# pema99/rust-path-tracer

Hardware: AMD Instinct MI355X
Metric: Mrays/s (higher is better)
Workload: dtype f32

## Files before the change

### rust-path-tracer_amd/csrc/k_traverse_nearest.h

```cpp
#ifndef RPT_K_TRAVERSE_NEAREST_H
#define RPT_K_TRAVERSE_NEAREST_H

#include "k_path.h"
#include "k_walk_stream.h"

template <int STACK, int THREADS>
__global__ __launch_bounds__(THREADS) void k_traverse_nearest(DevScene sc, DevState st, DevQueues q, uint32_t iteration) {
    __shared__ uint32_t lds_stack[THREADS / RPT_WAVE][STACK][RPT_WAVE];
    if (q.count[Q_DRAINED] != 0u) return;
    const uint32_t slot = blockIdx.x * THREADS + threadIdx.x;
    if (slot == 0u) {
        iteration_bookkeeping(q, iteration);
    }
    bool pending = false;
    if (slot < st.n_slots) pending = __float_as_uint(st.hit[slot].y) == HIT_PENDING;
    const SceneViewGlobal view{{sc.tri_isect}, sc.nodes};
    unsigned long long active = rpt_ballot(pending);
    if (active == 0ull) return;
    if (__lane_id() == (uint32_t)__ffsll((long long)active) - 1u) {
        raise_flag(&q.count[Q_ALIVE0 + (iteration & 1u) * Q_LINE]);
        atomicAdd(&q.ray_shards[(blockIdx.x % RPT_STAT_SHARDS) * RPT_STAT_STRIDE], (unsigned long long)__popcll(active));
    }
    if (!pending) return;
    float4 ra = st.ray_a[slot];
    float2 rb = st.ray_b[slot];
    F3 ro = f3(ra.x, ra.y, ra.z), rd = f3(ra.w, rb.x, rb.y);
    uint32_t *stack = &lds_stack[threadIdx.x / RPT_WAVE][0][threadIdx.x % RPT_WAVE];
    HitRecord h = traverse_one<STACK, false>(view, sc.fastdiv_ok, ro, rd, 0.0f, stack);
    store_hit(st, slot, h);
}

#define RPT_NEAREST_PLAIN 0
#define RPT_NEAREST_LAST 1
#define RPT_NEAREST_FIRST 2
template <int STACK, int THREADS, int MODE = RPT_NEAREST_PLAIN>
__attribute__((amdgpu_num_sgpr(RPT_LDS_WALK_SGPRS)))
__global__ __launch_bounds__(THREADS) void k_traverse_nearest_stream(DevScene sc, DevState st, DevQueues q, uint32_t iteration,
                                                                       uint32_t SPAN ,
                                                                       float cam_x, float cam_y, float cam_z ,
                                                                       DevConfig cfg, uint32_t gen_samples ,
                                                                       DevStats *stats) {
    constexpr bool LAST = MODE == RPT_NEAREST_LAST, FIRST = MODE == RPT_NEAREST_FIRST;
    constexpr uint32_t NW = THREADS / RPT_WAVE;
    __shared__ uint16_t lds_stack[NW][STACK][RPT_WAVE];
    __shared__ WgPool pool;
    float4 *lds_scene = rpt_lds_dyn;
    if (q.count[Q_DRAINED] != 0u) return;
    uint32_t *global_next = &q.count[Q_POOL0 + (iteration & 1u) * Q_LINE];
    if (blockIdx.x == 0u && threadIdx.x == 0u) {
        iteration_bookkeeping(q, iteration);
        q.count[Q_POOL0 + ((iteration + 1u) & 1u) * Q_LINE] = 0u;
    }
    const uint32_t lane = __lane_id(), wave = threadIdx.x / RPT_WAVE;
    if (threadIdx.x == 0u) {
        const uint32_t g = atomicAdd(global_next, SPAN);
        pool.word = wg_pool_span(g, SPAN, st.n_slots);
        pool.lock = 0u;
    }
    __syncthreads();
    if ((uint32_t)(pool.word >> 32) == 0u) return;
    if (LAST)
        for (uint32_t k = threadIdx.x; k < sc.last_flip_vecs; k += THREADS) lds_scene[sc.lds_vecs + k] = sc.lds_image_last[k];
    if (FIRST) {
        const uint32_t P2 = 2u * sc.lds_pairs;
        for (uint32_t k = threadIdx.x; k < 3u * P2; k += THREADS) {
            const float4 v = sc.lds_image[k];
            const float o = k < P2 ? cam_x : (k < 2u * P2 ? cam_y : cam_z);
            lds_scene[k] = make_float4(v.x - o, v.y - o, v.z - o, v.w - o);
        }
        for (uint32_t k = 3u * P2 + threadIdx.x; k < sc.lds_vecs; k += THREADS) lds_scene[k] = sc.lds_image[k];
        __syncthreads();
    }
    const SceneViewLds view = FIRST ? SceneViewLds{lds_scene, sc.lds_pairs, sc.n_triangles, sc.lds_root} : stage_scene_lds<THREADS>(sc, lds_scene);
    const float4 *img_lane = view.img;
    uint32_t stop_first = 0u;
    float order_bias = 0.0f;
    uint16_t *stack = &lds_stack[wave][0][lane];
    F3 ro = f3(0, 0, 0), rd = f3(1, 1, 1), ird = f3(1, 1, 1);
    LdsWalk w;
    walk_begin(view, w);
    w.cur = SceneViewLds::dead();
    uint32_t slot = 0u;
    bool have = false;
    bool pool_open = true;
    uint32_t traced = 0u;
    const bool done_here = LAST && q.implicit_zero != 0u;
    auto last_finish = [&](uint32_t s, const HitRecord &r, uint32_t stopped) -> bool {
        if (!done_here) {
            store_hit(st, s, r);
            return false;
        }
        if (r.tri == HIT_MISS) return true;
        if (stopped == 0u) {
            const uint32_t m = __float_as_uint(sc.tri_shade[4u * (r.tri & 0x7fffffffu) + 2u].w);
            const float4 e4 = sc.textured != 0u ? sc.materials[6u * m] : sc.mat_lite[2u * m];
            if ((e4.x != 0.0f || e4.y != 0.0f || e4.z != 0.0f) && (r.tri >> 31) == 0u) {
                const float4 tf = st.thr[s];
                finish_from_zero(st, s, mask_nan3(f3(tf.x, tf.y, tf.z) * f3(e4.x, e4.y, e4.z)));
                return false;
            }
        }
        set_hit_word(st, s, HIT_DONE_ZERO);
        return false;
    };
    auto last_park = [&](bool park, uint32_t s) {
        const uint32_t shard = (s >> q.sky_shard_shift) % RPT_Q_SHARDS;
        unsigned long long todo_m = rpt_ballot(park);
        while (todo_m != 0ull) {
            const uint32_t leader = (uint32_t)__ffsll((long long)todo_m) - 1u;
            const uint32_t sh = (uint32_t)__builtin_amdgcn_readlane((int)shard, (int)leader);
            const bool mine = park && shard == sh;
            const unsigned long long same = rpt_ballot(mine);
            uint32_t e = 0u;
            if (lane == leader) e = atomicAdd(&q.sky_cnt[sh * RPT_Q_SHARD_STRIDE], (uint32_t)__popcll(same));
            e = (uint32_t)__builtin_amdgcn_readlane((int)e, (int)leader);
            if (mine) {
                e += rpt_lane_rank(same);
                q.sky[q_position(sh, e)] = s;
                set_hit_word(st, s, HIT_PARKED);
            }
            todo_m &= ~same;
        }
    };
    for (;;) {
        const unsigned long long idle_m = rpt_ballot(walk_dead(w));
        const uint32_t n_idle = (uint32_t)__popcll(idle_m);
        if (pool_open && n_idle >= (uint32_t)RPT_STREAM_REFILL) {
            uint32_t base = 0u, got = 0u;
            bool finished = false;
            if (lane == 0u) base = wg_pool_take(&pool, global_next, st.n_slots, SPAN, n_idle, got, finished);
            base = (uint32_t)__builtin_amdgcn_readfirstlane((int)base);
            got = (uint32_t)__builtin_amdgcn_readfirstlane((int)got);
            pool_open = __builtin_amdgcn_readfirstlane((int)finished) == 0;
            bool took = false;
            if (LAST) {
                const bool writes = walk_dead(w) && have;
                bool park = false;
                if (writes) {
                    park = last_finish(slot, w.res, stop_first);
                    have = false;
                }
                if (done_here) last_park(park, slot);
            }
            if (walk_dead(w)) {
                if (!LAST && have) {
                    store_hit(st, slot, w.res);
                    have = false;
                }
                const uint32_t rank = rpt_lane_rank(idle_m);
                if (rank < got) {
                    const uint32_t cand = base + rank;
                    const uint32_t word = __float_as_uint(st.hit[cand].y);
                    bool pending;
                    if (FIRST && gen_samples != 0u) {
                        pending = begin_first_path(st, cfg, stats, cand, word, gen_samples, ro, rd);
                    } else {
                        pending = word == HIT_PENDING;
                        if (pending) {
                            const float4 ra = st.ray_a[cand];
                            const float2 rb = st.ray_b[cand];
                            ro = f3(ra.x, ra.y, ra.z); rd = f3(ra.w, rb.x, rb.y);
                        }
                    }
                    if (pending) {
                        slot = cand;
                        took = true;
                        if (fastdiv_ray_ok(sc.fastdiv_ok, ro, rd)) {
                            ird = f3(rptm::rcp_rn_window(rd.x), rptm::rcp_rn_window(rd.y), rptm::rcp_rn_window(rd.z));
                            walk_begin(view, w);
                            have = true;
                            if (LAST) {
                                bool may_emit = false;
                                for (uint32_t e = 0; e < sc.last_emit_n; ++e) {
                                    float t_e;
                                    bool bf_e;
                                    may_emit = moller_trumbore_view(view, sc.last_emit_tri[e], ro, rd, t_e, bf_e) || may_emit;
                                }
                                stop_first = may_emit ? 0u : 1u;
                                const bool flipped = !may_emit && sc.last_flip_vecs != 0u;
                                img_lane = flipped ? view.img + sc.lds_vecs : view.img;
                                order_bias = flipped ? __builtin_inff() : 0.0f;
                            }
                        } else {
                            LdsWalk alone;
                            walk_begin(view, alone);
                            lds_walk_run<STACK, false, false, false, false, FIRST>(view, alone, ro, rd, rd, 0.0f, stack, 0x7fffffff);
                            if (LAST) {
                                w.res = alone.res;
                                stop_first = 0u;
                                have = true;
                            } else {
                                store_hit(st, cand, alone.res);
                            }
                        }
                    }
                }
            }
            traced += (uint32_t)__popcll(rpt_ballot(took));
            if (got != 0u || !pool_open) continue;
            if (idle_m == ~0ull) { __builtin_amdgcn_s_sleep(8); continue; }
        }
        if (idle_m == ~0ull) {
            if (!pool_open) break;
            continue;
        }
        if (LAST) lds_walk_run<STACK, false, true, false, true>(view, w, ro, rd, ird, 0.0f, stack, pool_open ? RPT_STREAM_TRIPS : 0x7fffffff, img_lane, stop_first, order_bias);
        else lds_walk_run<STACK, false, true, false, false, FIRST>(view, w, ro, rd, ird, 0.0f, stack, pool_open ? RPT_STREAM_TRIPS : 0x7fffffff);
    }
    if (LAST) {
        bool park = false;
        if (have) park = last_finish(slot, w.res, stop_first);
        if (done_here) last_park(park, slot);
    } else if (have) {
        store_hit(st, slot, w.res);
    }
    if (lane == 0u && traced != 0u) {
        raise_flag(&q.count[Q_ALIVE0 + (iteration & 1u) * Q_LINE]);
        atomicAdd(&q.ray_shards[(blockIdx.x % RPT_STAT_SHARDS) * RPT_STAT_STRIDE], (unsigned long long)traced);
    }
}

template <int STACK, int WIDTH , bool COOP >
__attribute__((amdgpu_waves_per_eu(gstream_waves(STACK, WIDTH, COOP), 8)))
 __global__ __launch_bounds__(RPT_WAVE) void k_traverse_nearest_gstream(DevScene sc, DevState st, DevQueues q, uint32_t iteration,
                                                                       uint32_t SPAN ) {
    __shared__ WaveStack<STACK, WIDTH> lds_stack;
    __shared__ uint16_t pend[RPT_WAVE * gstream_rays_nearest(STACK, WIDTH)];
    if (q.count[Q_DRAINED] != 0u) return;
    const uint32_t lane = threadIdx.x;
    if (blockIdx.x == 0u && lane == 0u) {
        iteration_bookkeeping(q, iteration);
    }
    const uint32_t span_begin = blockIdx.x * SPAN;
    if (span_begin >= st.n_slots) return;
    const uint32_t span_end = span_begin + SPAN < st.n_slots ? span_begin + SPAN : st.n_slots;
    uint32_t count = 0u;
    for (uint32_t base = span_begin; base < span_end; base += RPT_WAVE) {
        const uint32_t s = base + lane;
        const bool p = s < span_end && __float_as_uint(st.hit[s].y) == HIT_PENDING;
        const unsigned long long m = rpt_ballot(p);
        if (p) pend[count + rpt_lane_rank(m)] = (uint16_t)(s - span_begin);
        count += (uint32_t)__popcll(m);
    }
    if (count == 0u) return;
    __builtin_amdgcn_fence(__ATOMIC_RELEASE, "wavefront");
    __builtin_amdgcn_wave_barrier();
    if (lane == 0u) {
        raise_flag(&q.count[Q_ALIVE0 + (iteration & 1u) * Q_LINE]);
        atomicAdd(&q.ray_shards[(blockIdx.x % RPT_STAT_SHARDS) * RPT_STAT_STRIDE], (unsigned long long)count);
    }
    typedef SceneViewPairsT<COOP> View;
    const View view{{sc.tri_isect}, sc.gpairs, sc.glinks};
    auto stack = lds_stack.column(lane);
    F3 ro = f3(0, 0, 0), rd = f3(1, 1, 1), ird = f3(1, 1, 1);
    Walk<View> w;
    walk_begin(view, w);
    w.cur = View::dead();
    uint32_t slot = 0u, next = 0u;
    bool have = false;
    const uint32_t refill_at = iteration == 0u ? (uint32_t)RPT_GSTREAM_REFILL_FIRST : (uint32_t)RPT_GSTREAM_REFILL;
    for (;;) {
        const unsigned long long idle_m = rpt_ballot(walk_dead(w));
        const uint32_t n_idle = (uint32_t)__popcll(idle_m);
        const bool more = next < count;
        if ((more && n_idle >= refill_at) || idle_m == ~0ull) {
            if (walk_dead(w)) {
                if (have) {
                    store_hit(st, slot, w.res);
                    have = false;
                }
                const uint32_t at = next + rpt_lane_rank(idle_m);
                if (at < count) {
                    slot = span_begin + pend[at];
                    const float4 ra = st.ray_a[slot];
                    const float2 rb = st.ray_b[slot];
                    ro = f3(ra.x, ra.y, ra.z); rd = f3(ra.w, rb.x, rb.y);
                    have = true;
                    if (fastdiv_ray_ok(sc.fastdiv_ok, ro, rd)) {
                        ird = f3(rptm::rcp_rn_window(rd.x), rptm::rcp_rn_window(rd.y), rptm::rcp_rn_window(rd.z));
                        walk_begin(view, w);
                    } else {
                        w.res = traverse_loop<STACK, false, false>(view, ro, rd, rd, 0.0f, stack);
                    }
                }
            }
            if (!more) break;
            next += n_idle;
            continue;
        }
        walk_run<STACK, false, true>(view, w, ro, rd, ird, 0.0f, stack, more ? RPT_GSTREAM_TRIPS : 0x7fffffff);
    }
}

#endif
```

### rust-path-tracer_amd/csrc/k_traverse_shadow_kernels.h

```cpp
template <int STACK, int THREADS>
__global__ __launch_bounds__(THREADS) void RPT_SHADOW_KERNEL(k_traverse_shadow)(DevScene sc, DevState st, DevQueues q, DevConfig cfg, DevStats *stats) {
    constexpr bool SEGMENT = RPT_SHADOW_KERNEL_SEGMENT;
    __shared__ uint32_t lds_stack[THREADS / RPT_WAVE][STACK][RPT_WAVE];
    if (q.count[Q_DRAINED] != 0u) return;
    uint32_t i = blockIdx.x * THREADS + threadIdx.x;
    uint32_t positions, n;
    q_extent(q.shadow_cnt, positions, n);
    if (i == 0u && n) atomicAdd(&stats->shadow_rays, (unsigned long long)n);
    if (blockIdx.x * THREADS >= positions) return;
    const SceneViewGlobal view{{sc.tri_isect}, sc.nodes};
    if (i >= positions || !q_filled(q.shadow_cnt, i)) return;
    float4 o = q.sh_o[i], d = q.sh_d[i];
    uint32_t tag = __float_as_uint(d.w);
    uint32_t *stack = &lds_stack[threadIdx.x / RPT_WAVE][0][threadIdx.x % RPT_WAVE];
    HitRecord h = traverse_one<STACK, true, SEGMENT>(view, sc.fastdiv_ok, f3(o.x, o.y, o.z), f3(d.x, d.y, d.z), SEGMENT ? shadow_segment_bound(o.w) : o.w, stack);
    shadow_resolve(st, q, cfg, i, tag, h.tri == HIT_MISS);
}

template <int STACK, int THREADS, bool FIXED >
__attribute__((amdgpu_num_sgpr(RPT_LDS_WALK_SGPRS)))
__global__ __launch_bounds__(THREADS) void RPT_SHADOW_KERNEL(k_traverse_shadow_stream)(DevScene sc, DevState st, DevQueues q, DevStats *stats, uint32_t SPAN) {
    constexpr bool SEGMENT = RPT_SHADOW_KERNEL_SEGMENT;
    constexpr uint32_t NW = THREADS / RPT_WAVE;
    __shared__ uint16_t lds_stack[NW][STACK][RPT_WAVE];
    __shared__ WgPool pool;
    float4 *lds_scene = rpt_lds_dyn;
    if (q.count[Q_DRAINED] != 0u) return;
    uint32_t n, n_entries;
    q_extent(q.shadow_cnt, n, n_entries);
    uint32_t *global_next = &q.count[Q_SPOOL];
    if (blockIdx.x == 0u && threadIdx.x == 0u && n_entries) atomicAdd(&stats->shadow_rays, (unsigned long long)n_entries);
    const uint32_t lane = __lane_id(), wave = threadIdx.x / RPT_WAVE;
    if (threadIdx.x == 0u) {
        const uint32_t g = n ? atomicAdd(global_next, SPAN) : 0u;
        pool.word = wg_pool_span(g, SPAN, n);
        pool.lock = 0u;
    }
    __syncthreads();
    if ((uint32_t)(pool.word >> 32) == 0u) return;
    const SceneViewLds view = stage_scene_lds<THREADS>(sc, lds_scene, FIXED);
    uint16_t *stack = &lds_stack[wave][0][lane];
    F3 ro = f3(0, 0, 0), rd = f3(1, 1, 1), ird = f3(1, 1, 1);
    float max_t = 0.0f;
    LdsWalk w;
    walk_begin(view, w);
    w.cur = SceneViewLds::dead();
    uint32_t entry = 0u;
    bool have = false;
    bool pool_open = true;
    for (;;) {
        const unsigned long long idle_m = rpt_ballot(walk_dead(w));
        const uint32_t n_idle = (uint32_t)__popcll(idle_m);
        if (pool_open && n_idle >= (uint32_t)RPT_STREAM_REFILL) {
            uint32_t base = 0u, got = 0u;
            bool finished = false;
            if (lane == 0u) base = wg_pool_take(&pool, global_next, n, SPAN, n_idle, got, finished);
            base = (uint32_t)__builtin_amdgcn_readfirstlane((int)base);
            got = (uint32_t)__builtin_amdgcn_readfirstlane((int)got);
            pool_open = __builtin_amdgcn_readfirstlane((int)finished) == 0;
            if (walk_dead(w)) {
                if (have) {
                    q.sh_c[entry].w = w.res.tri == HIT_MISS ? 0.0f : 1.0f;
                    have = false;
                }
                const uint32_t rank = rpt_lane_rank(idle_m);
                if (rank < got && q_filled(q.shadow_cnt, base + rank)) {
                    entry = base + rank;
                    const float4 o = q.sh_o[entry], d = q.sh_d[entry];
                    ro = f3(o.x, o.y, o.z); rd = f3(d.x, d.y, d.z);
                    max_t = SEGMENT ? shadow_segment_bound(o.w) : o.w;
                    have = true;
                    if (fastdiv_ray_ok(sc.fastdiv_ok, ro, rd)) {
                        ird = f3(rptm::rcp_rn_window(rd.x), rptm::rcp_rn_window(rd.y), rptm::rcp_rn_window(rd.z));
                        walk_begin(view, w);
                    } else {
                        w.res = traverse_loop<STACK, true, false, FIXED, SEGMENT>(view, ro, rd, rd, max_t, stack);
                    }
                }
            }
            if (got != 0u || !pool_open) continue;
            if (idle_m == ~0ull) { __builtin_amdgcn_s_sleep(8); continue; }
        }
        if (idle_m == ~0ull) {
            if (!pool_open) break;
            continue;
        }
        lds_walk_run<STACK, true, true, FIXED, false, false, SEGMENT>(view, w, ro, rd, ird, max_t, stack, pool_open ? RPT_STREAM_TRIPS : 0x7fffffff);
    }
    if (have) q.sh_c[entry].w = w.res.tri == HIT_MISS ? 0.0f : 1.0f;
}

template <int STACK, int WIDTH, bool COOP, bool FIXED >
__attribute__((amdgpu_waves_per_eu(gstream_waves(STACK, WIDTH, COOP), 8)))
 __global__ __launch_bounds__(RPT_WAVE) void RPT_SHADOW_KERNEL(k_traverse_shadow_gstream)(DevScene sc, DevState st, DevQueues q, DevConfig cfg, DevStats *stats,
                                                                      uint32_t SPAN) {
    constexpr bool SEGMENT = RPT_SHADOW_KERNEL_SEGMENT;
    __shared__ WaveStack<STACK, WIDTH> lds_stack;
    __shared__ uint8_t occluded[RPT_WAVE * RPT_GSTREAM_RAYS];
    if (q.count[Q_DRAINED] != 0u) return;
    const uint32_t lane = threadIdx.x;
    uint32_t n, n_entries;
    q_extent(q.shadow_cnt, n, n_entries);
    if (blockIdx.x == 0u && lane == 0u && n_entries) atomicAdd(&stats->shadow_rays, (unsigned long long)n_entries);
    const uint32_t begin = blockIdx.x * SPAN;
    if (begin >= n) return;
    const uint32_t end = begin + SPAN < n ? begin + SPAN : n;
    {
        typedef SceneViewPairsT<COOP> View;
        const View view = FIXED ? View{{sc.tri_isect}, sc.gpairs_shadow, sc.glinks_shadow} : View{{sc.tri_isect}, sc.gpairs, sc.glinks};
        auto stack = lds_stack.column(lane);
        F3 ro = f3(0, 0, 0), rd = f3(1, 1, 1), ird = f3(1, 1, 1);
        float max_t = 0.0f;
        Walk<View> w;
        walk_begin(view, w);
        w.cur = View::dead();
        uint32_t entry = 0u, next = begin;
        bool have = false;
        for (;;) {
            const unsigned long long idle_m = rpt_ballot(walk_dead(w));
            const uint32_t n_idle = (uint32_t)__popcll(idle_m);
            const bool more = next < end;
            if ((more && n_idle >= (uint32_t)RPT_GSTREAM_REFILL) || idle_m == ~0ull) {
                if (walk_dead(w)) {
                    if (have) {
                        occluded[entry - begin] = w.res.tri == HIT_MISS ? (uint8_t)0 : (uint8_t)1;
                        have = false;
                    }
                    const uint32_t at = next + rpt_lane_rank(idle_m);
                    if (at < end && q_filled(q.shadow_cnt, at)) {
                        const float4 o = q.sh_o[at], d = q.sh_d[at];
                        ro = f3(o.x, o.y, o.z); rd = f3(d.x, d.y, d.z);
                        max_t = SEGMENT ? shadow_segment_bound(o.w) : o.w;
                        entry = at;
                        have = true;
                        if (fastdiv_ray_ok(sc.fastdiv_ok, ro, rd)) {
                            ird = f3(rptm::rcp_rn_window(rd.x), rptm::rcp_rn_window(rd.y), rptm::rcp_rn_window(rd.z));
                            walk_begin(view, w);
                        } else {
                            w.res = traverse_loop<STACK, true, false, FIXED, SEGMENT>(view, ro, rd, rd, max_t, stack);
                        }
                    }
                }
                if (!more) break;
                next += n_idle;
                continue;
            }
            walk_run<STACK, true, true, FIXED, SEGMENT>(view, w, ro, rd, ird, max_t, stack, more ? RPT_GSTREAM_TRIPS : 0x7fffffff);
        }
    }
    __builtin_amdgcn_fence(__ATOMIC_RELEASE, "wavefront");
    __builtin_amdgcn_wave_barrier();
    for (uint32_t base = begin; base < end; base += RPT_WAVE) {
        const uint32_t e = base + lane;
        if (e < end && q_filled(q.shadow_cnt, e)) shadow_resolve(st, q, cfg, e, __float_as_uint(q.sh_d[e].w), occluded[e - begin] == 0u);
    }
}

template <int STACK, bool ANY_HIT, bool LDS_SCENE, int THREADS>
__global__ __launch_bounds__(THREADS) void RPT_SHADOW_KERNEL(k_trace_debug)(DevScene sc, uint32_t n, const float *origins, const float *dirs,
                                                         const float *max_t, float *out_t, uint32_t *out_tri, uint32_t *out_flags) {
    constexpr bool SEGMENT = RPT_SHADOW_KERNEL_SEGMENT && ANY_HIT;
    typedef typename StackElem<LDS_SCENE>::type StackT;
    __shared__ StackT lds_stack[THREADS / RPT_WAVE][STACK][RPT_WAVE];
    float4 *lds_scene = rpt_lds_dyn;
    uint32_t i = blockIdx.x * THREADS + threadIdx.x;
    const auto view = stage_scene<LDS_SCENE, THREADS>(sc, lds_scene);
    if (i >= n) return;
    F3 ro = f3(origins[3 * i], origins[3 * i + 1], origins[3 * i + 2]);
    F3 rd = f3(dirs[3 * i], dirs[3 * i + 1], dirs[3 * i + 2]);
    StackT *stack = &lds_stack[threadIdx.x / RPT_WAVE][0][threadIdx.x % RPT_WAVE];
    HitRecord h = traverse_one<STACK, ANY_HIT, SEGMENT>(view, sc.fastdiv_ok, ro, rd, ANY_HIT ? (SEGMENT ? shadow_segment_bound(max_t[i]) : max_t[i]) : 0.0f, stack);
    out_t[i] = h.t;
    out_tri[i] = (h.tri == HIT_MISS) ? 0u : (h.tri & 0x7fffffffu);
    out_flags[i] = (h.tri == HIT_MISS) ? 0u : (1u | ((h.tri >> 31) << 1));
}
```

### rust-path-tracer_amd/csrc/k_walk.h

```cpp
#ifndef RPT_K_WALK_H
#define RPT_K_WALK_H

#include <type_traits>

#include "k_common.h"
#include "rpt_fastdiv.h"

template <bool SMALL> struct StackElem { typedef uint32_t type; };
template <> struct StackElem<true> { typedef uint16_t type; };
template <typename T> __device__ __forceinline__ void stack_put(T *s, int sp, uint32_t v) { s[sp * RPT_WAVE] = (T)v; }
template <typename T> __device__ __forceinline__ uint32_t stack_get(T *s, int sp) { return (uint32_t)s[sp * RPT_WAVE]; }
struct Stack24 {
    uint16_t *lo;
    uint8_t *hi;
};
__device__ __forceinline__ void stack_put(Stack24 s, int sp, uint32_t v) {
    s.lo[sp * RPT_WAVE] = (uint16_t)v;
    s.hi[sp * RPT_WAVE] = (uint8_t)(v >> 16);
}
__device__ __forceinline__ uint32_t stack_get(Stack24 s, int sp) { return (uint32_t)s.lo[sp * RPT_WAVE] | ((uint32_t)s.hi[sp * RPT_WAVE] << 16); }
template <int K> struct StackBits {
    uint16_t *lo;
    uint32_t hi[K];
};
// ... 148 lines not shown
    }
};

struct SceneViewLds {
    static constexpr bool kCoopLeaves = false;
    const float4 *img;
    uint32_t pairs, tris, root_desc;
    typedef uint32_t Cur;
    __device__ __forceinline__ Cur root() const { return root_desc; }
    __device__ __forceinline__ static bool is_inner(Cur c) { return c < LDS_DESC_DEAD; }
    __device__ __forceinline__ static bool is_leaf(Cur c) { return c >= LDS_DESC_LEAF; }
    __device__ __forceinline__ static Cur dead() { return LDS_DESC_DEAD; }
    __device__ __forceinline__ static bool is_dead(Cur c) { return c == LDS_DESC_DEAD; }
    __device__ __forceinline__ const float4 *tri_base() const { return img + 6u * pairs + ((pairs + 3u) >> 2); }
    __device__ __forceinline__ void edges(uint32_t ti, F3 &e1, F3 &e2) const {
        const float4 *t = tri_base() + 3u * ti;
        e1 = xyz4(t[1]); e2 = xyz4(t[2]);
    }
    __device__ __forceinline__ F3 corner(uint32_t ti) const { return xyz4(tri_base()[3u * ti]); }
};
template <typename T> __device__ __forceinline__ T lds_at(const float4 *base, uint32_t bytes) {
    return *reinterpret_cast<const T *>(reinterpret_cast<const char *>(base) + bytes);
}
__device__ __forceinline__ float4 lds_planes(const float4 *base, uint32_t desc) {
#if defined(__HIP_DEVICE_COMPILE__)
    typedef const __attribute__((address_space(3))) float4 *LdsVec;
    const uint32_t b = (uint32_t)(LdsVec)base;
    uint32_t a;
    asm("v_lshl_add_u32 %0, %1, 2, %2" : "=v"(a) : "v"(desc), "v"(b));
    return *(LdsVec)a;
#else
    return lds_at<float4>(base, desc << 2);
#endif
}
constexpr uint32_t LDS_STACK_STRIDE = RPT_WAVE * (uint32_t)sizeof(uint16_t);
__device__ __forceinline__ uint32_t lds_stack_address(const uint16_t *stack) {
#if defined(__HIP_DEVICE_COMPILE__)
    return (uint32_t)(const __attribute__((address_space(3))) uint16_t *)stack;
#else
    return 0u;
#endif
}
__device__ __forceinline__ void lds_stack_store(uint32_t at, uint32_t v) {
#if defined(__HIP_DEVICE_COMPILE__)
    *(__attribute__((address_space(3))) uint16_t *)at = (uint16_t)v;
#endif
}
__device__ __forceinline__ uint32_t lds_stack_load(uint32_t at) {
#if defined(__HIP_DEVICE_COMPILE__)
    return *(const __attribute__((address_space(3))) uint16_t *)at;
#else
    return 0u;
#endif
}

template <typename Corner>
__device__ __forceinline__ bool moller_trumbore(F3 edge1, F3 edge2, Corner corner, F3 ro, F3 rd, float &out_t, bool &backface) {
    F3 pv = cross3(rd, edge2);
    float det = dot3(edge1, pv);
    backface = (rptm::f2u(det) >> 31) != 0u;
    if (rptm::absr(det) < 1e-6f) return false;
    float inv_det = rptm::rcp_rn(det);
    F3 tv = ro - corner();
    float u = dot3(tv, pv) * inv_det;
    if (u < 0.0f || u > 1.0f) return false;
    F3 qv = cross3(tv, edge1);
    float v = dot3(rd, qv) * inv_det;
    if (v < 0.0f || u + v > 1.0f) return false;
    float t = dot3(edge2, qv) * inv_det;
    if (t < 0.0f) return false;
    out_t = t;
    return true;
}
template <typename View>
__device__ __forceinline__ bool moller_trumbore_view(const View &view, uint32_t ti, F3 ro, F3 rd, float &out_t, bool &backface) {
    F3 edge1, edge2;
    view.edges(ti, edge1, edge2);
    return moller_trumbore(edge1, edge2, [&] { return view.corner(ti); }, ro, rd, out_t, backface);
}
__device__ __forceinline__ bool moller_trumbore_regs(F3 edge1, F3 edge2, F3 corner, F3 ro, F3 rd, float &out_t, bool &backface) {
    return moller_trumbore(edge1, edge2, [&] { return corner; }, ro, rd, out_t, backface);
}

__device__ __forceinline__ float rpt_readlane(float v, int lane) { return __uint_as_float((uint32_t)__builtin_amdgcn_readlane((int)__float_as_uint(v), lane)); }
__device__ __forceinline__ uint32_t rpt_readlane_u(uint32_t v, int lane) { return (uint32_t)__builtin_amdgcn_readlane((int)v, lane); }

__device__ __forceinline__ bool rpt_all_lanes_hold(uint32_t x, uint32_t x0) { return rpt_ballot(x == x0) == rpt_ballot(true); }

template <typename View> struct Walk {
    typename View::Cur cur;
    int sp;
    HitRecord res;
};
template <typename View>
__device__ __forceinline__ void walk_begin(const View &view, Walk<View> &w) {
    w.cur = view.root();
    w.sp = 0;
    w.res.t = 1000000.0f;
    w.res.tri = HIT_MISS;
}
template <typename View>
__device__ __forceinline__ bool walk_dead(const Walk<View> &w) { return View::is_dead(w.cur); }

template <bool ANY_HIT, typename View>
__device__ __forceinline__ typename View::Cur walk_pop(const View &view, uint32_t e) {
    if constexpr (View::kUniformScalar && !ANY_HIT && !View::kCoopLeaves) {
        const uint32_t e0 = (uint32_t)__builtin_amdgcn_readfirstlane((int)e);
        if (rpt_all_lanes_hold(e, e0)) return view.from_entry_uniform(e0);
        asm volatile("" ::: "memory");
        return view.from_entry(e);
    } else {
        return view.from_entry(e);
    }
}

__device__ __forceinline__ float shadow_segment_bound(float max_t) {
    if (!(max_t < 1000000.0f)) return max_t >= 1000000.0f ? 1000000.0f : max_t;
    if (max_t == 0.0f) return __uint_as_float(1u);
    const uint32_t b = __float_as_uint(max_t);
    return __uint_as_float(max_t > 0.0f ? b + 1u : b - 1u);
}

template <int STACK, bool ANY_HIT, bool FAST, bool FIXED = false, bool SEGMENT = false , typename View, typename StackRef>
__device__ __forceinline__ void walk_run(const View &view, Walk<View> &w, F3 ro, F3 rd, F3 ird, float max_t, StackRef &stack, int budget) {
    static_assert(!FIXED || ANY_HIT, "only the any-hit walk may choose its order");
    static_assert(!SEGMENT || ANY_HIT, "only a shadow ray is a segment");
    typedef typename View::Cur Cur;
    HitRecord res = w.res;
    int sp = w.sp;
    Cur cur = w.cur;
    for (int trip = 0; trip < budget; ++trip) {
        const bool at_inner = View::is_inner(cur);
        const bool at_leaf = View::is_leaf(cur);
        const unsigned long long inner_m = rpt_ballot(at_inner), leaf_m = rpt_ballot(at_leaf);
        if ((inner_m | leaf_m) == 0ull) break;
        if (at_inner && (uint32_t)__popcll(leaf_m) <= (uint32_t)__popcll(inner_m)) {
            float4 lmin, lmax, rmin, rmax;
            float tl, tr;
            bool hit_l, hit_r;
            if constexpr (View::kUniformScalar) {
                const uint32_t c0 = (uint32_t)__builtin_amdgcn_readfirstlane((int)cur);
                if (rpt_all_lanes_hold(cur, c0)) {
                    view.children_uniform(c0, lmin, lmax, rmin, rmax);
                    hit_l = slab_test<FAST>(lmin, lmax, ro, rd, ird, SEGMENT ? max_t : res.t, tl);
                    hit_r = slab_test<FAST>(rmin, rmax, ro, rd, ird, SEGMENT ? max_t : res.t, tr);
                    asm volatile("" : "+v"(tl), "+v"(tr));
                } else {
                    asm volatile("" ::: "memory");
                    view.children(cur, lmin, lmax, rmin, rmax);
                    hit_l = slab_test<FAST>(lmin, lmax, ro, rd, ird, SEGMENT ? max_t : res.t, tl);
                    hit_r = slab_test<FAST>(rmin, rmax, ro, rd, ird, SEGMENT ? max_t : res.t, tr);
                }
            } else {
                view.children(cur, lmin, lmax, rmin, rmax);
                hit_l = slab_test<FAST>(lmin, lmax, ro, rd, ird, SEGMENT ? max_t : res.t, tl);
                hit_r = slab_test<FAST>(rmin, rmax, ro, rd, ird, SEGMENT ? max_t : res.t, tr);
            }
            const bool swap = FIXED ? (hit_r && !hit_l) : (hit_r && (!hit_l || tl > tr));
            if (hit_l || hit_r) {
                if (hit_l && hit_r && sp < STACK) {
                    stack_put(stack, sp, view.far_entry(cur, swap));
                    sp += 1;
                }
                cur = View::enter(swap, lmin, lmax, rmin, rmax);
            } else if (sp == 0) {
                cur = View::dead();
            } else {
                sp -= 1;
                cur = walk_pop<ANY_HIT>(view, stack_get(stack, sp));
            }
        }
        const bool do_leaf = (uint32_t)__popcll(leaf_m) > (uint32_t)__popcll(inner_m);
        if (do_leaf) {
            bool accepted = false, coop_done = false;
            const uint32_t count = View::leaf_count(cur), first = View::leaf_first(cur);
            if constexpr (View::kCoopLeaves) {
                const bool fat = at_leaf && count > (uint32_t)RPT_COOP_LEAF_MIN;
                unsigned long long todo = rpt_ballot(fat);
                if (todo != 0ull) {
                    const unsigned long long exec_m = rpt_ballot(true);
                    const uint32_t n_act = (uint32_t)__popcll(exec_m);
                    const uint32_t my_rank = rpt_lane_rank(exec_m);
                    coop_done = fat;
                    do {
                        const int lead = __ffsll((long long)todo) - 1;
                        const uint32_t b_count = rpt_readlane_u(count, lead), b_first = rpt_readlane_u(first, lead);
                        const unsigned long long group = rpt_ballot(fat && first == b_first && count == b_count) & todo;
                        todo &= ~group;
                        for (uint32_t base = 0; base < b_count; base += n_act) {
                            const bool mine = base + my_rank < b_count;
                            const uint32_t ti = b_first + base + my_rank;
                            F3 e1 = f3(0, 0, 0), e2 = f3(0, 0, 0), corner = f3(0, 0, 0);
                            if (mine) {
                                view.edges(ti, e1, e2);
                                corner = view.corner(ti);
                            }
                            unsigned long long g = ANY_HIT ? (group & ~rpt_ballot(accepted)) : group;
                            while (g != 0ull) {
                                const int L = __ffsll((long long)g) - 1;
                                g &= g - 1ull;
                                const F3 bo = f3(rpt_readlane(ro.x, L), rpt_readlane(ro.y, L), rpt_readlane(ro.z, L));
                                const F3 bd = f3(rpt_readlane(rd.x, L), rpt_readlane(rd.y, L), rpt_readlane(rd.z, L));
                                const float b_max = ANY_HIT ? rpt_readlane(max_t, L) : 0.0f;
                                uint32_t best_bits = __float_as_uint(rpt_readlane(res.t, L));
                                uint32_t best_tri = HIT_MISS;
                                float t = 0.0f;
                                bool bf = false;
                                const bool acc = mine && moller_trumbore_regs(e1, e2, corner, bo, bd, t, bf) && t > 0.001f &&
                                                 __float_as_uint(t) < best_bits && (!ANY_HIT || (SEGMENT ? t < b_max : t <= b_max));
                                unsigned long long am = rpt_ballot(acc);
                                while (am != 0ull) {
                                    const int l = __ffsll((long long)am) - 1;
                                    am &= am - 1ull;
                                    const uint32_t tb = __float_as_uint(rpt_readlane(t, l));
                                    if (tb < best_bits) {
                                        best_bits = tb;
                                        best_tri = rpt_readlane_u(ti, l) | (rpt_readlane_u(bf ? 1u : 0u, l) << 31);
                                        if (ANY_HIT) break;
                                    }
                                }
                                if ((int)__lane_id() == L && best_tri != HIT_MISS) {
                                    res.t = __uint_as_float(best_bits);
                                    res.tri = best_tri;
                                    accepted = true;
                                }
                            }
                        }
                    } while (todo != 0ull);
                }
            }
            if (at_leaf && !coop_done) {
                bool leaf_uniform = false;
                uint32_t c0 = 0u;
                if constexpr (View::kUniformScalar && !ANY_HIT && !View::kCoopLeaves) {
                    c0 = (uint32_t)__builtin_amdgcn_readfirstlane((int)cur);
                    leaf_uniform = rpt_all_lanes_hold(cur, c0);
                    if (leaf_uniform) {
                        const uint32_t n0 = View::leaf_count(c0), f0 = View::leaf_first(c0);
                        for (uint32_t i = 0; i < n0; ++i) {
                            const uint32_t ti = f0 + i;
                            F3 e1, e2, a;
                            view.triangle_uniform(ti, e1, e2, a);
                            float t = 0.0f;
                            bool bf = false;
                            if (moller_trumbore_regs(e1, e2, a, ro, rd, t, bf) && t > 0.001f && t < res.t) {
                                asm volatile("" ::: "memory");
                                res.t = t;
                                res.tri = ti | (bf ? 0x80000000u : 0u);
                            }
                        }
                    }
                }
                if (!leaf_uniform) {
                asm volatile("" ::: "memory");
                for (uint32_t i = 0; i < count; ++i) {
                    uint32_t ti = first + i;
                    float t = 0.0f;
                    bool bf = false;
                    if (moller_trumbore_view(view, ti, ro, rd, t, bf) && t > 0.001f && (SEGMENT ? t < max_t : (t < res.t && (!ANY_HIT || t <= max_t)))) {
                        asm volatile("" ::: "memory");
                        res.t = t;
                        res.tri = ti | (bf ? 0x80000000u : 0u);
                        if (ANY_HIT) { accepted = true; break; }
                    }
                }
                }
            }
            if (at_leaf) {
                if ((ANY_HIT && accepted) || sp == 0) {
                    cur = View::dead();
                } else {
                    sp -= 1;
                    cur = walk_pop<ANY_HIT>(view, stack_get(stack, sp));
                }
            }
        }
    }
    w.cur = cur;
    w.sp = sp;
    w.res = res;
}

template <bool SIGNED>
__device__ __forceinline__ bool slab_pair_lds(float n_x, float n_y, float n_z, float f_x, float f_y, float f_z, F3 ro, F3 rd, F3 ird,
                                              float prev_min_t, float &tmin_out) {
    float tmin, tmax;
    if (SIGNED) {
        float a = rptm::div_by_rcp(n_x - ro.x, rd.x, ird.x), b = rptm::div_by_rcp(n_y - ro.y, rd.y, ird.y), c = rptm::div_by_rcp(n_z - ro.z, rd.z, ird.z);
        float d = rptm::div_by_rcp(f_x - ro.x, rd.x, ird.x), e = rptm::div_by_rcp(f_y - ro.y, rd.y, ird.y), f = rptm::div_by_rcp(f_z - ro.z, rd.z, ird.z);
        tmin = __builtin_fmaxf(__builtin_fmaxf(a, b), c);
        tmax = __builtin_fminf(__builtin_fminf(d, e), f);
    } else {
        float tx1 = (n_x - ro.x) / rd.x, tx2 = (f_x - ro.x) / rd.x;
        float ty1 = (n_y - ro.y) / rd.y, ty2 = (f_y - ro.y) / rd.y;
        float tz1 = (n_z - ro.z) / rd.z, tz2 = (f_z - ro.z) / rd.z;
        slab_interval(tx1, tx2, ty1, ty2, tz1, tz2, tmin, tmax);
    }
    tmin_out = tmin;
    return tmax >= tmin && tmax > 0.0f && tmin < prev_min_t;
}

typedef Walk<SceneViewLds> LdsWalk;

template <int STACK, bool ANY_HIT, bool SIGNED, bool FIXED = false, bool MIXED = false, bool PRESUB = false, bool SEGMENT = false >
__device__ __forceinline__ void lds_walk_run(const SceneViewLds &view, LdsWalk &w, F3 ro, F3 rd, F3 ird, float max_t, uint16_t *stack,
                                             int budget, const float4 *img_lane = nullptr, uint32_t stop_first = 0u, float order_bias = 0.0f) {
    static_assert(!FIXED || ANY_HIT, "only the any-hit walk may choose its order");
    static_assert(!MIXED || (!ANY_HIT && !FIXED), "MIXED is the nearest-hit walk with per-lane early exits");
    static_assert(!SEGMENT || ANY_HIT, "only a shadow ray is a segment");
    const F3 ro_slab = PRESUB ? f3(0.0f, 0.0f, 0.0f) : ro;
    const uint32_t P = view.pairs;
    const float4 *img = MIXED ? img_lane : view.img;
    const float4 *px = img + ((SIGNED && rd.x < 0.0f) ? P : 0u);
    const float4 *py = img + 2u * P + ((SIGNED && rd.y < 0.0f) ? P : 0u);
    const float4 *pz = img + 4u * P + ((SIGNED && rd.z < 0.0f) ? P : 0u);
    const float4 *descs = img + 6u * P;
    uint32_t cur = w.cur;
    const uint32_t bottom = lds_stack_address(stack), limit = bottom + (uint32_t)STACK * LDS_STACK_STRIDE;
    uint32_t top = bottom + (uint32_t)w.sp;
    HitRecord res = w.res;
    for (int trip = 0; trip < budget; ++trip) {
        const bool at_inner = SceneViewLds::is_inner(cur);
        const bool at_leaf = SceneViewLds::is_leaf(cur);
        const unsigned long long inner_m = rpt_ballot(at_inner), leaf_m = rpt_ballot(at_leaf);
        if ((inner_m | leaf_m) == 0ull) break;
        uint32_t n_leaf = (uint32_t)__popcll(leaf_m), n_inner = (uint32_t)__popcll(inner_m);
        asm("" : "+s"(n_leaf), "+s"(n_inner));
        const bool do_leaf = n_leaf > n_inner;
        if (at_inner && !do_leaf) {
            const float4 X = SIGNED ? lds_planes(px, cur) : lds_at<float4>(px, cur << 2), Y = SIGNED ? lds_planes(py, cur) : lds_at<float4>(py, cur << 2),
                         Z = SIGNED ? lds_planes(pz, cur) : lds_at<float4>(pz, cur << 2);
            const uint32_t d = lds_at<uint32_t>(descs, cur);
            float tl, tr;
            const bool hit_l = slab_pair_lds<SIGNED>(X.x, Y.x, Z.x, X.z, Y.z, Z.z, ro_slab, rd, ird, SEGMENT ? max_t : res.t, tl);
            const bool hit_r = slab_pair_lds<SIGNED>(X.y, Y.y, Z.y, X.w, Y.w, Z.w, ro_slab, rd, ird, SEGMENT ? max_t : res.t, tr);
            const bool swap = FIXED ? (hit_r && !hit_l)
                            : MIXED ? (hit_r && (!hit_l || tl > tr + order_bias))
                                    : (hit_r && (!hit_l || tl > tr));
            if (hit_l || hit_r) {
                const uint32_t nf = __builtin_amdgcn_alignbit(d, d, swap ? 16u : 0u);
                if (hit_l && hit_r && top < limit) {
                    lds_stack_store(top, nf >> 16);
                    top += LDS_STACK_STRIDE;
                }
                cur = nf & 0xffffu;
            } else if (top == bottom) {
                cur = LDS_DESC_DEAD;
            } else {
                top -= LDS_STACK_STRIDE;
                cur = lds_stack_load(top);
            }
        }
        if (at_leaf && do_leaf) {
            bool accepted = false;
            const uint32_t count = (cur >> 9) & 63u, first = cur & 511u;
            const float4 *rec = view.tri_base() + 3u * first;
            for (uint32_t ti = first, end = first + count; ti != end; ++ti, rec += 3) {
                float t;
                bool bf = false;
                if (moller_trumbore(xyz4(rec[1]), xyz4(rec[2]), [&] { return xyz4(rec[0]); }, ro, rd, t, bf) && t > 0.001f && (SEGMENT ? t < max_t : (t < res.t && (!ANY_HIT || t <= max_t)))) {
                    asm volatile("" ::: "memory");
                    res.t = t;
                    res.tri = ti | (bf ? 0x80000000u : 0u);
                    if (ANY_HIT || (MIXED && stop_first != 0u)) { accepted = true; break; }
                }
            }
            if (((ANY_HIT || MIXED) && accepted) || top == bottom) {
                cur = LDS_DESC_DEAD;
            } else {
                top -= LDS_STACK_STRIDE;
                cur = lds_stack_load(top);
            }
        }
    }
    w.cur = cur;
    w.sp = (int)(top - bottom);
    w.res = res;
}

template <int STACK, bool ANY_HIT, bool FAST, bool FIXED = false, bool SEGMENT = false, typename View, typename StackRef>
__device__ __forceinline__ HitRecord traverse_loop(const View &view, F3 ro, F3 rd, F3 ird, float max_t, StackRef &stack) {
    Walk<View> w;
    walk_begin(view, w);
    if constexpr (std::is_same<View, SceneViewLds>::value) lds_walk_run<STACK, ANY_HIT, FAST, FIXED, false, false, SEGMENT>(view, w, ro, rd, ird, max_t, stack, 0x7fffffff);
    else walk_run<STACK, ANY_HIT, FAST, FIXED, SEGMENT>(view, w, ro, rd, ird, max_t, stack, 0x7fffffff);
    return w.res;
}

__device__ __forceinline__ bool fastdiv_ray_ok(uint32_t fastdiv_ok, F3 ro, F3 rd) {
    return fastdiv_ok != 0u && rptm::fastdiv_divisor_ok(rd.x) && rptm::fastdiv_divisor_ok(rd.y) && rptm::fastdiv_divisor_ok(rd.z) &&
           rptm::fastdiv_operand_ok(ro.x) && rptm::fastdiv_operand_ok(ro.y) && rptm::fastdiv_operand_ok(ro.z);
}

template <int STACK, bool ANY_HIT, bool SEGMENT = false, typename View, typename StackT>
__device__ __forceinline__ HitRecord traverse_one(const View &view, uint32_t fastdiv_ok, F3 ro, F3 rd, float max_t, StackT *stack) {
    if (fastdiv_ray_ok(fastdiv_ok, ro, rd)) {
        F3 ird = f3(rptm::rcp_rn_window(rd.x), rptm::rcp_rn_window(rd.y), rptm::rcp_rn_window(rd.z));
        return traverse_loop<STACK, ANY_HIT, true, false, SEGMENT>(view, ro, rd, ird, max_t, stack);
    }
    return traverse_loop<STACK, ANY_HIT, false, false, SEGMENT>(view, ro, rd, rd, max_t, stack);
}

#endif
```

Before: 13300.

## Add wave-coherent streaming LDS walk with sentinel stack and majority leaf/inner scheduling

```diff
diff --git a/rust-path-tracer_amd/csrc/k_traverse_nearest.h b/rust-path-tracer_amd/csrc/k_traverse_nearest.h
--- a/rust-path-tracer_amd/csrc/k_traverse_nearest.h
+++ b/rust-path-tracer_amd/csrc/k_traverse_nearest.h
@@ -76,6 +76,7 @@
     uint32_t stop_first = 0u;
     float order_bias = 0.0f;
     uint16_t *stack = &lds_stack[wave][0][lane];
+    lds_stream_stack_begin(stack);
     F3 ro = f3(0, 0, 0), rd = f3(1, 1, 1), ird = f3(1, 1, 1);
     LdsWalk w;
     walk_begin(view, w);
@@ -184,7 +185,7 @@
                         } else {
                             LdsWalk alone;
                             walk_begin(view, alone);
-                            lds_walk_run<STACK, false, false, false, false, FIRST>(view, alone, ro, rd, rd, 0.0f, stack, 0x7fffffff);
+                            lds_walk_run<STACK - 1, false, false, false, FIRST>(view, alone, ro, rd, rd, 0.0f, lds_stream_stack_rest(stack), 0x7fffffff);
                             if (LAST) {
                                 w.res = alone.res;
                                 stop_first = 0u;
@@ -204,8 +205,8 @@
             if (!pool_open) break;
             continue;
         }
-        if (LAST) lds_walk_run<STACK, false, true, false, true>(view, w, ro, rd, ird, 0.0f, stack, pool_open ? RPT_STREAM_TRIPS : 0x7fffffff, img_lane, stop_first, order_bias);
-        else lds_walk_run<STACK, false, true, false, false, FIRST>(view, w, ro, rd, ird, 0.0f, stack, pool_open ? RPT_STREAM_TRIPS : 0x7fffffff);
+        if (LAST) lds_stream_walk_run<STACK, false, false, true>(view, w, ro, rd, ird, 0.0f, stack, pool_open ? RPT_STREAM_TRIPS : 0x7fffffff, img_lane, stop_first, order_bias);
+        else lds_stream_walk_run<STACK, false, false, false, FIRST>(view, w, ro, rd, ird, 0.0f, stack, pool_open ? RPT_STREAM_TRIPS : 0x7fffffff);
     }
     if (LAST) {
         bool park = false;
diff --git a/rust-path-tracer_amd/csrc/k_traverse_shadow_kernels.h b/rust-path-tracer_amd/csrc/k_traverse_shadow_kernels.h
--- a/rust-path-tracer_amd/csrc/k_traverse_shadow_kernels.h
+++ b/rust-path-tracer_amd/csrc/k_traverse_shadow_kernels.h
@@ -40,6 +40,7 @@
     if ((uint32_t)(pool.word >> 32) == 0u) return;
     const SceneViewLds view = stage_scene_lds<THREADS>(sc, lds_scene, FIXED);
     uint16_t *stack = &lds_stack[wave][0][lane];
+    lds_stream_stack_begin(stack);
     F3 ro = f3(0, 0, 0), rd = f3(1, 1, 1), ird = f3(1, 1, 1);
     float max_t = 0.0f;
     LdsWalk w;
@@ -74,7 +75,8 @@
                         ird = f3(rptm::rcp_rn_window(rd.x), rptm::rcp_rn_window(rd.y), rptm::rcp_rn_window(rd.z));
                         walk_begin(view, w);
                     } else {
-                        w.res = traverse_loop<STACK, true, false, FIXED, SEGMENT>(view, ro, rd, rd, max_t, stack);
+                        uint16_t *rest = lds_stream_stack_rest(stack);
+                        w.res = traverse_loop<STACK - 1, true, false, FIXED, SEGMENT>(view, ro, rd, rd, max_t, rest);
                     }
                 }
             }
@@ -85,7 +87,7 @@
             if (!pool_open) break;
             continue;
         }
-        lds_walk_run<STACK, true, true, FIXED, false, false, SEGMENT>(view, w, ro, rd, ird, max_t, stack, pool_open ? RPT_STREAM_TRIPS : 0x7fffffff);
+        lds_stream_walk_run<STACK, true, FIXED, false, false, SEGMENT>(view, w, ro, rd, ird, max_t, stack, pool_open ? RPT_STREAM_TRIPS : 0x7fffffff);
     }
     if (have) q.sh_c[entry].w = w.res.tri == HIT_MISS ? 0.0f : 1.0f;
 }
diff --git a/rust-path-tracer_amd/csrc/k_walk.h b/rust-path-tracer_amd/csrc/k_walk.h
--- a/rust-path-tracer_amd/csrc/k_walk.h
+++ b/rust-path-tracer_amd/csrc/k_walk.h
@@ -474,15 +474,13 @@
 
 typedef Walk<SceneViewLds> LdsWalk;
 
-template <int STACK, bool ANY_HIT, bool SIGNED, bool FIXED = false, bool MIXED = false, bool PRESUB = false, bool SEGMENT = false >
-__device__ __forceinline__ void lds_walk_run(const SceneViewLds &view, LdsWalk &w, F3 ro, F3 rd, F3 ird, float max_t, uint16_t *stack,
-                                             int budget, const float4 *img_lane = nullptr, uint32_t stop_first = 0u, float order_bias = 0.0f) {
+template <int STACK, bool ANY_HIT, bool SIGNED, bool FIXED = false, bool PRESUB = false, bool SEGMENT = false >
+__device__ __forceinline__ void lds_walk_run(const SceneViewLds &view, LdsWalk &w, F3 ro, F3 rd, F3 ird, float max_t, uint16_t *stack, int budget) {
     static_assert(!FIXED || ANY_HIT, "only the any-hit walk may choose its order");
-    static_assert(!MIXED || (!ANY_HIT && !FIXED), "MIXED is the nearest-hit walk with per-lane early exits");
     static_assert(!SEGMENT || ANY_HIT, "only a shadow ray is a segment");
     const F3 ro_slab = PRESUB ? f3(0.0f, 0.0f, 0.0f) : ro;
     const uint32_t P = view.pairs;
-    const float4 *img = MIXED ? img_lane : view.img;
+    const float4 *img = view.img;
     const float4 *px = img + ((SIGNED && rd.x < 0.0f) ? P : 0u);
     const float4 *py = img + 2u * P + ((SIGNED && rd.y < 0.0f) ? P : 0u);
     const float4 *pz = img + 4u * P + ((SIGNED && rd.z < 0.0f) ? P : 0u);
@@ -506,9 +504,7 @@
             float tl, tr;
             const bool hit_l = slab_pair_lds<SIGNED>(X.x, Y.x, Z.x, X.z, Y.z, Z.z, ro_slab, rd, ird, SEGMENT ? max_t : res.t, tl);
             const bool hit_r = slab_pair_lds<SIGNED>(X.y, Y.y, Z.y, X.w, Y.w, Z.w, ro_slab, rd, ird, SEGMENT ? max_t : res.t, tr);
-            const bool swap = FIXED ? (hit_r && !hit_l)
-                            : MIXED ? (hit_r && (!hit_l || tl > tr + order_bias))
-                                    : (hit_r && (!hit_l || tl > tr));
+            const bool swap = FIXED ? (hit_r && !hit_l) : (hit_r && (!hit_l || tl > tr));
             if (hit_l || hit_r) {
                 const uint32_t nf = __builtin_amdgcn_alignbit(d, d, swap ? 16u : 0u);
                 if (hit_l && hit_r && top < limit) {
@@ -534,10 +530,10 @@
                     asm volatile("" ::: "memory");
                     res.t = t;
                     res.tri = ti | (bf ? 0x80000000u : 0u);
-                    if (ANY_HIT || (MIXED && stop_first != 0u)) { accepted = true; break; }
-                }
-            }
-            if (((ANY_HIT || MIXED) && accepted) || top == bottom) {
+                    if (ANY_HIT) { accepted = true; break; }
+                }
+            }
+            if ((ANY_HIT && accepted) || top == bottom) {
                 cur = LDS_DESC_DEAD;
             } else {
                 top -= LDS_STACK_STRIDE;
@@ -550,11 +546,108 @@
     w.res = res;
 }
 
+constexpr uint32_t LDS_DESC_POP = LDS_DESC_DEAD + 1u;
+__device__ __forceinline__ void lds_stream_stack_begin(uint16_t *stack) { stack[0] = (uint16_t)LDS_DESC_DEAD; }
+__device__ __forceinline__ uint16_t *lds_stream_stack_rest(uint16_t *stack) { return stack + RPT_WAVE; }
+
+__device__ __forceinline__ bool moller_trumbore_flat(F3 edge1, F3 edge2, F3 corner, F3 ro, F3 rd, float &out_t, float &out_det) {
+    const F3 pv = cross3(rd, edge2);
+    const float det = dot3(edge1, pv);
+    const float inv_det = rptm::rcp_rn(det);
+    const F3 tv = ro - corner;
+    const float u = dot3(tv, pv) * inv_det;
+    const F3 qv = cross3(tv, edge1);
+    const float v = dot3(rd, qv) * inv_det;
+    float lo = rptm::fminr(u, v), hi = rptm::fmaxr(u, u + v), t = dot3(edge2, qv) * inv_det;
+    asm volatile("" : "+v"(lo), "+v"(hi), "+v"(t));
+    out_t = t;
+    out_det = det;
+    return !(rptm::absr(det) < 1e-6f) & !(lo < 0.0f) & !(hi > 1.0f);
+}
+
+template <int STACK, bool ANY_HIT, bool FIXED = false, bool MIXED = false, bool PRESUB = false, bool SEGMENT = false >
+__device__ __forceinline__ void lds_stream_walk_run(const SceneViewLds &view, LdsWalk &w, F3 ro, F3 rd, F3 ird, float max_t, uint16_t *stack ,
+                                                    int budget, const float4 *img_lane = nullptr, uint32_t stop_first = 0u, float order_bias = 0.0f) {
+    static_assert(!FIXED || ANY_HIT, "only the any-hit walk may choose its order");
+    static_assert(!MIXED || (!ANY_HIT && !FIXED), "MIXED is the nearest-hit walk with per-lane early exits");
+    static_assert(!SEGMENT || ANY_HIT, "only a shadow ray is a segment");
+    const F3 ro_slab = PRESUB ? f3(0.0f, 0.0f, 0.0f) : ro;
+    const uint32_t P = view.pairs;
+    const float4 *img = MIXED ? img_lane : view.img;
+    const float4 *px = img + (rd.x < 0.0f ? P : 0u);
+    const float4 *py = img + 2u * P + (rd.y < 0.0f ? P : 0u);
+    const float4 *pz = img + 4u * P + (rd.z < 0.0f ? P : 0u);
+    const float4 *descs = img + 6u * P;
+    uint32_t cur = w.cur;
+    const uint32_t bottom = lds_stack_address(stack) + LDS_STACK_STRIDE, limit = bottom + (uint32_t)(STACK - 1) * LDS_STACK_STRIDE;
+    uint32_t top = bottom + (uint32_t)w.sp;
+    HitRecord res = w.res;
+    uint32_t left = (uint32_t)budget;
+    uint32_t n_leaf = (uint32_t)__popcll(rpt_ballot(SceneViewLds::is_leaf(cur))), n_inner = (uint32_t)__popcll(rpt_ballot(SceneViewLds::is_inner(cur)));
+    asm("" : "+s"(n_leaf), "+s"(n_inner));
+    uint32_t go;
+    do {
+        if (n_leaf > n_inner) {
+            if (SceneViewLds::is_leaf(cur)) {
+                bool accepted = false;
+                const uint32_t first = cur & 511u;
+                uint32_t ti = first;
+                const uint32_t end = first + ((cur >> 9) & 63u);
+                const float4 *rec = view.tri_base() + 3u * first;
+                do {
+                    float t, det;
+                    const bool ok = moller_trumbore_flat(xyz4(rec[1]), xyz4(rec[2]), xyz4(rec[0]), ro, rd, t, det);
+                    if (ok && t > 0.001f && (SEGMENT ? t < max_t : (t < res.t && (!ANY_HIT || t <= max_t)))) {
+                        asm volatile("" ::: "memory");
+                        res.t = t;
+                        res.tri = ti | (rptm::f2u(det) & 0x80000000u);
+                        if (ANY_HIT || (MIXED && stop_first != 0u)) { accepted = true; break; }
+                    }
+                    ++ti;
+                    rec += 3;
+                } while (ti != end);
+                cur = ((ANY_HIT || MIXED) && accepted) ? LDS_DESC_DEAD : LDS_DESC_POP;
+            }
+        }
+        if (n_leaf <= n_inner) {
+            if (SceneViewLds::is_inner(cur)) {
+                const float4 X = lds_planes(px, cur), Y = lds_planes(py, cur), Z = lds_planes(pz, cur);
+                const uint32_t d = lds_at<uint32_t>(descs, cur);
+                float tl, tr;
+                const bool hit_l = slab_pair_lds<true>(X.x, Y.x, Z.x, X.z, Y.z, Z.z, ro_slab, rd, ird, SEGMENT ? max_t : res.t, tl);
+                const bool hit_r = slab_pair_lds<true>(X.y, Y.y, Z.y, X.w, Y.w, Z.w, ro_slab, rd, ird, SEGMENT ? max_t : res.t, tr);
+                const bool swap = FIXED ? (hit_r && !hit_l)
+                                : MIXED ? (hit_r && (!hit_l || tl > tr + order_bias))
+                                        : (hit_r && (!hit_l || tl > tr));
+                const uint32_t nf = __builtin_amdgcn_alignbit(d, d, swap ? 16u : 0u);
+                if (hit_l && hit_r && top < limit) {
+                    lds_stack_store(top, nf >> 16);
+                    top += LDS_STACK_STRIDE;
+                }
+                cur = (hit_l || hit_r) ? (nf & 0xffffu) : LDS_DESC_POP;
+            }
+        }
+        if (cur == LDS_DESC_POP) {
+            top -= LDS_STACK_STRIDE;
+            cur = lds_stack_load(top);
+        }
+        --left;
+        n_leaf = (uint32_t)__popcll(rpt_ballot(SceneViewLds::is_leaf(cur)));
+        n_inner = (uint32_t)__popcll(rpt_ballot(SceneViewLds::is_inner(cur)));
+        asm("" : "+s"(n_leaf), "+s"(n_inner));
+        go = n_leaf + n_inner;
+        go = go < left ? go : left;
+    } while (go != 0u);
+    w.cur = cur;
+    w.sp = (int)(top - bottom);
+    w.res = res;
+}
+
 template <int STACK, bool ANY_HIT, bool FAST, bool FIXED = false, bool SEGMENT = false, typename View, typename StackRef>
 __device__ __forceinline__ HitRecord traverse_loop(const View &view, F3 ro, F3 rd, F3 ird, float max_t, StackRef &stack) {
     Walk<View> w;
     walk_begin(view, w);
-    if constexpr (std::is_same<View, SceneViewLds>::value) lds_walk_run<STACK, ANY_HIT, FAST, FIXED, false, false, SEGMENT>(view, w, ro, rd, ird, max_t, stack, 0x7fffffff);
+    if constexpr (std::is_same<View, SceneViewLds>::value) lds_walk_run<STACK, ANY_HIT, FAST, FIXED, false, SEGMENT>(view, w, ro, rd, ird, max_t, stack, 0x7fffffff);
     else walk_run<STACK, ANY_HIT, FAST, FIXED, SEGMENT>(view, w, ro, rd, ird, max_t, stack, 0x7fffffff);
     return w.res;
 }
```

Measured after the change: 13750, median of 6. 1.03x the previous value.
